# GetOverMassif/QSP-SLAM

Measured on AMD Instinct MI355X. Metric: joint-opt iters/sec (BA+SDF), higher is better.
Workload: dtype f32 as 2 x fp16 per operand (hi + 2^-11 lo'), 3 fp16 products per multiply-add, f32 accumulate (decoder); f64 (bundle adjustment)

## Files before the change

qsp_slam_amd/csrc/sdf_mlp.hpp:

```cpp
#pragma once
#include <hip/hip_runtime.h>
#include <stdint.h>

namespace qsp {

typedef float f32x16 __attribute__((ext_vector_type(16)));

#ifndef QSP_EXP_VARIANT
#define QSP_EXP_VARIANT 0
#endif
#if (QSP_EXP_VARIANT & 16)
__device__ unsigned long long qsp_dbg_ts[96];
__device__ unsigned long long qsp_dbg_rt[96];
__device__ int qsp_dbg_n;
#define QSP_TS()                                                                        \
    if (blockIdx.x == 0 && blockIdx.y == 0 && threadIdx.x == 0 && ts_n < 96) {          \
        qsp_dbg_rt[ts_n] = __builtin_amdgcn_s_memrealtime();                            \
        qsp_dbg_ts[ts_n++] = __builtin_readcyclecounter();                              \
        qsp_dbg_n = ts_n;                                                               \
    }
#define QSP_TSK(i)                                                                      \
    if (blockIdx.x == 0 && threadIdx.x == 0 && tsk_first) {                             \
        qsp_dbg_rt[80 + (i)] = __builtin_amdgcn_s_memrealtime();                        \
        qsp_dbg_ts[80 + (i)] = __builtin_readcyclecounter();                            \
    }
#else
#define QSP_TS()
#define QSP_TSK(i)
#endif

constexpr int TILE_P = 64;
constexpr int HID = 512;
constexpr int CODE_LEN = 64;
constexpr int NIN = CODE_LEN + 3;
constexpr int SKIP_COL = HID - NIN;
constexpr int K4 = SKIP_COL + 3;
constexpr int KG4 = K4 / 8;
constexpr int K0_PAD = 96;
constexpr int LDA = HID + 4;
constexpr int LDST = 68;
constexpr int STASH_SHIFT = 1;
static_assert((SKIP_COL - STASH_SHIFT) % 4 == 0 && STASH_SHIFT + NIN <= LDST, "stash row: aligned quads of units 444.., 67 inputs");
constexpr int LDJ = 96;
constexpr int NJ = 72;
constexpr int MLP_THREADS = 512;
constexpr int HT_TILES = 6;

struct MlpParams {
    const float4* wf[8];
    const float4* wb[8];
    const float* bias[8];
    const float* w8;
    float b8;
    const float* w0c;
    const float* w4c;
    const float4* w0x;
    const float4* wf3[8];
    const float4* wb3[8];
    const float4* wfh[8];
    const float4* wbh[8];
    const float4* wbh4s;
    int* range_flag;
    int use_tanh;
    int narrow;
    uint8_t skip[8];
    uint8_t ks_in[8];
    uint8_t ks_out[8];
    uint8_t ncb_in[8];
    uint8_t ncb_out[8];
};

__device__ __forceinline__ float mlp_output(float t, int use_tanh, float& dy) {
    float y = tanhf(t);
    dy = 1.f - y * y;
    if (use_tanh) {
        const float y2 = tanhf(y);
        dy = (1.f - y2 * y2) * dy;
        y = y2;
    }
    return y;
}

struct __attribute__((aligned(16))) MlpSmem {
    float act[TILE_P * LDA];
    float stash[TILE_P * LDST];
    float xin[TILE_P * 4];
    float code[CODE_LEN];
    float c0[HID];
    float c4[HID];
    float y[TILE_P];
    float red[8 * TILE_P];
    float rscale[TILE_P];
    float rres[TILE_P];
    float w8[HID];
    float dy[TILE_P];
};

template <bool AG>
__device__ __forceinline__ f32x16 mfma32t(float a, float b, f32x16 c) {
    if (AG) {
        asm("v_mfma_f32_32x32x2_f32 %0, %1, %2, %0" : "+a"(c) : "v"(a), "v"(b));
        return c;
    }
    return __builtin_amdgcn_mfma_f32_32x32x2f32(a, b, c, 0, 0, 0);
}
template <bool AG>
__device__ __forceinline__ void mfma_acc_settle(f32x16& c0, f32x16& c1, f32x16& c2, f32x16& c3) {
    if (AG) asm volatile("s_nop 15\n\ts_nop 7" : "+a"(c0), "+a"(c1), "+a"(c2), "+a"(c3));
}
template <bool AG>
__device__ __forceinline__ void mfma_acc_settle(f32x16& c0) {
    if (AG) asm volatile("s_nop 15\n\ts_nop 7" : "+a"(c0));
}

__device__ __forceinline__ int acc_row(int i, int lane) { return (i & 3) + 8 * (i >> 2) + 4 * (lane >> 5); }

typedef float f32x4 __attribute__((ext_vector_type(4)));
typedef const __attribute__((address_space(1))) f32x4* gptr4;

__device__ __forceinline__ f32x4 lds4(const float* p) { return *reinterpret_cast<const f32x4*>(p); }

#define QSP_MFMA_STEP_2x2(a0, a1, b0, b1)                   \
    acc[0][0] = mfma32t<AG>(b0.x, a0.x, acc[0][0]);         \
    acc[0][1] = mfma32t<AG>(b1.x, a0.x, acc[0][1]);              \
    acc[1][0] = mfma32t<AG>(b0.x, a1.x, acc[1][0]);              \
    acc[1][1] = mfma32t<AG>(b1.x, a1.x, acc[1][1]);              \
    acc[0][0] = mfma32t<AG>(b0.y, a0.y, acc[0][0]);              \
    acc[0][1] = mfma32t<AG>(b1.y, a0.y, acc[0][1]);              \
    acc[1][0] = mfma32t<AG>(b0.y, a1.y, acc[1][0]);              \
    acc[1][1] = mfma32t<AG>(b1.y, a1.y, acc[1][1]);              \
    acc[0][0] = mfma32t<AG>(b0.z, a0.z, acc[0][0]);              \
    acc[0][1] = mfma32t<AG>(b1.z, a0.z, acc[0][1]);              \
    acc[1][0] = mfma32t<AG>(b0.z, a1.z, acc[1][0]);              \
    acc[1][1] = mfma32t<AG>(b1.z, a1.z, acc[1][1]);              \
    acc[0][0] = mfma32t<AG>(b0.w, a0.w, acc[0][0]);              \
    acc[0][1] = mfma32t<AG>(b1.w, a0.w, acc[0][1]);              \
    acc[1][0] = mfma32t<AG>(b0.w, a1.w, acc[1][0]);              \
    acc[1][1] = mfma32t<AG>(b1.w, a1.w, acc[1][1]);

template <int PF>
struct WRing {
    f32x4 q0[PF], q1[PF];
};

template <int PF>
__device__ __forceinline__ void ring_prime(WRing<PF>& R, const float4* __restrict__ w0_, const float4* __restrict__ w1_, int lane) {
    gptr4 w0 = (gptr4)w0_;
    gptr4 w1 = (gptr4)w1_;
#pragma unroll
    for (int d = 0; d < PF; ++d) {
        R.q0[d] = w0[d * 64 + lane];
        R.q1[d] = w1[d * 64 + lane];
    }
}

struct BiasQuads {
    f32x4 v[2][4];
};

template <int KG, int PF, bool BIAS, bool AG>
__device__ __forceinline__ void gemm_2x2(const float* __restrict__ act, const float4* __restrict__ w0_,
                                         const float4* __restrict__ w1_, const float4* __restrict__ n0_,
                                         const float4* __restrict__ n1_, WRing<PF>& R, f32x16 (&acc)[2][2], int lane,
                                         const float* __restrict__ bias_wave, BiasQuads& bq) {
    static_assert(KG % PF == 0 && KG >= 2 * PF, "KG must be a multiple of the prefetch depth, at least twice it");
    gptr4 w0 = (gptr4)w0_;
    gptr4 w1 = (gptr4)w1_;
    gptr4 n0 = (gptr4)n0_;
    gptr4 n1 = (gptr4)n1_;
    const float* a_row0 = act + (lane & 31) * LDA + 4 * (lane >> 5);
    const float* a_row1 = a_row0 + 32 * LDA;
    f32x4 a0 = lds4(a_row0), a1 = lds4(a_row1);
#pragma nounroll
    for (int kg = 0; kg < KG - PF; kg += PF) {
#pragma unroll
        for (int d = 0; d < PF; ++d) {
            const f32x4 b0 = R.q0[d], b1 = R.q1[d];
#if (QSP_EXP_VARIANT & 8)
            R.q0[d] = w0[((kg + d + PF) & 15) * 64 + lane];
            R.q1[d] = w1[((kg + d + PF) & 15) * 64 + lane];
#elif (QSP_EXP_VARIANT & 4)
            R.q0[d] = w0[d * 64 + lane];
            R.q1[d] = w1[d * 64 + lane];
#elif !(QSP_EXP_VARIANT & 1)
            R.q0[d] = w0[(kg + d + PF) * 64 + lane];
            R.q1[d] = w1[(kg + d + PF) * 64 + lane];
#endif
#if !(QSP_EXP_VARIANT & 2)
            const f32x4 a0n = lds4(a_row0 + 8 * (kg + d + 1));
            const f32x4 a1n = lds4(a_row1 + 8 * (kg + d + 1));
#else
            const f32x4 a0n = a1, a1n = a0;
#endif
            __builtin_amdgcn_sched_barrier(0);
            QSP_MFMA_STEP_2x2(a0, a1, b0, b1)
            __builtin_amdgcn_sched_barrier(0);
            a0 = a0n;
            a1 = a1n;
        }
    }
    if (BIAS) {
        typedef const __attribute__((address_space(1))) f32x4* gq;
        gq bp = (gq)(bias_wave + 4 * (lane >> 5));
#pragma unroll
        for (int c = 0; c < 2; ++c)
#pragma unroll
            for (int g = 0; g < 4; ++g) bq.v[c][g] = bp[(32 * c + 8 * g) / 4];
    }
#pragma unroll
    for (int d = 0; d < PF; ++d) {
        const f32x4 b0 = R.q0[d], b1 = R.q1[d];
#if !(QSP_EXP_VARIANT & 1)
        R.q0[d] = n0[d * 64 + lane];
        R.q1[d] = n1[d * 64 + lane];
// ... 1110 lines not shown
            for (int j = 0; j < 8; ++j)
                pa[j & 3] = fmaf(fmaf((float)lo[j], 0.00048828125f, (float)hi[j]), j < 4 ? w0[j] : w1[j - 4], pa[j & 3]);
        }
        const float part = (pa[0] + pa[1]) + (pa[2] + pa[3]);
        if (lane < TP) s.red[wave * TP + lane] = part;
    }
    __syncthreads();
    if (tid < TP) {
        float t = P.b8;
#pragma unroll
        for (int q = 0; q < 4; ++q) t += s.red[q * TP + tid];
        float dy_;
        s.y[tid] = mlp_output(t, P.use_tanh, dy_);
        s.dy[tid] = dy_;
    }
    __syncthreads();
    QSP_HTS()
#ifdef QSP_H2_STAMPS
    if (threadIdx.x == 0 && blockIdx.x == 0) qsp_h2_nts = hts_n;
#endif
    if constexpr (BWD) {
        const bool seed_full = NARROW && P.skip[7];
#pragma unroll
        for (int r = 0; r < NR; ++r) {
            const int p = 32 * r + (lane & 31);
            const float dy = s.dy[p];
#pragma unroll
            for (int c = 0; c < NCB; ++c)
#pragma unroll
                for (int g = 0; g < 4; ++g) {
                    const int u0 = 32 * NCB * wave + 32 * c + 8 * g + 4 * h;
                    if (seed_full) {
                        const f32x4 wv = lds4(s.w8 + u0);
                        f32x4 v;
#pragma unroll
                        for (int q = 0; q < 4; ++q) v[q] = h2_mask_sel(dy * wv[q], mk[7][r][c >> 1], (c & 1) * 16 + 4 * g + q);
                        h2_store4(img, p, u0, v, amax);
                    } else {
                        f16x4 m;
#pragma unroll
                        for (int q = 0; q < 4; ++q) m[q] = (_Float16)h2_mask_sel(1.f, mk[7][r][c >> 1], (c & 1) * 16 + 4 * g + q);
                        *reinterpret_cast<f16x4*>(img + h2_at(p, u0)) = m;
                    }
                }
        }
        if (!NARROW) ringh_prime(ring, QSP_WBH(7), CS, lane);
        __syncthreads();
#define QSP_BWDH(L, KS_, NWB)                                                                                            \
  if (!(NARROW && P.skip[L])) {         \
    const bool act_ = !NARROW || cb0 < (int)P.ncb_in[L];                                                                  \
    const int cu0_ = 32 * NCB * wave;                                                                                    \
    (void)cu0_;                                                                                                          \
    _Pragma("unroll") for (int r_ = 0; r_ < NR; ++r_) _Pragma("unroll") for (int c_ = 0; c_ < NCB; ++c_)                 \
        _Pragma("unroll") for (int i_ = 0; i_ < 16; ++i_) { acc[r_][c_][i_] = 0.f; acc2[r_][c_][i_] = 0.f; }             \
    if constexpr (NARROW)                                                                                                \
        gemm_h2<KS_, PF, NCB, NR, false, false, true, (L) == 7>(img, QSP_WBH(L), CS, QSP_WBH(L), CS, ring, acc, acc2, lane,    \
                                                                act_ ? min((int)P.ks_out[L], KS_) : 0);                  \
    else                                                                                                                 \
        gemm_h2<KS_, PF, NCB, NR, HAND, true, false, (L) == 7>(img, QSP_WBH(L), CS, NWB, CS, ring, acc, acc2, lane);       \
    QSP_PIN_ACC()                                                                                                        \
    __syncthreads();                                                                                                     \
    float dyr_[NR];                                                   \
    _Pragma("unroll") for (int r_ = 0; r_ < NR; ++r_) dyr_[r_] = (L) == 7 ? s.dy[32 * r_ + (lane & 31)] : 1.f;           \
    _Pragma("unroll") for (int c_ = 0; c_ < NCB; ++c_) _Pragma("unroll") for (int g_ = 0; g_ < 4; ++g_) {                \
        const int u0_ = 32 * NCB * wave + 32 * c_ + 8 * g_ + 4 * h;                                                      \
        _Pragma("unroll") for (int r_ = 0; r_ < NR; ++r_) {                                                              \
            const int p_ = 32 * r_ + (lane & 31);                                                                      \
            f32x4 v_, raw_;                                                                                              \
            _Pragma("unroll") for (int q_ = 0; q_ < 4; ++q_) {                                                           \
                float x_ = fmaf(acc2[r_][c_][4 * g_ + q_], 0.00048828125f, acc[r_][c_][4 * g_ + q_]);                   \
                if ((L) == 7) x_ *= dyr_[r_];                                                                            \
                raw_[q_] = x_;                                                                                           \
                const float m_ = h2_mask_sel(x_, mk[(L) - 1][r_][c_ >> 1], (c_ & 1) * 16 + 4 * g_ + q_);                       \
                v_[q_] = m_;                                                                                             \
            }                                                                                                            \
             \
             \
             \
            if (!NARROW && (L) == 4 && cu0_ + 32 * c_ + 32 > SKIP_COL) {                 \
                if (u0_ + 3 >= SKIP_COL) *reinterpret_cast<f32x4*>(s.stash + p_ * LDST + (u0_ - (SKIP_COL - STASH_SHIFT))) = raw_; \
            }                                                                                                            \
            h2_store4(img, p_, u0_, v_, amax);                                                                           \
        }                                                                                                                \
        __builtin_amdgcn_sched_barrier(0);                                                                               \
    }                                                                                                                    \
    if (!NARROW && (L) > 1) ringh_prime(ring, NWB, CS, lane);      \
    __syncthreads();                                                                                                     \
  }
        QSP_BWDH(7, KSH, QSP_WBH(6))
        QSP_BWDH(6, KSH, QSP_WBH(5))
        QSP_BWDH(5, KSH, QSP_WBH(4))
        if constexpr (NARROW) {
            f32x4 sk[NR][4];
            gemm_side_h2<PF, NR, NW, NARROW>(img, P.wbh4s, wave, lane, sk, NARROW ? (int)P.ks_out[4] : KSH);
            const int c0 = side_c0<NR, NW>(wave);
#pragma unroll
            for (int r = 0; r < NR; ++r) {
                if (r >= side_count<NR, NW>(wave)) break;
                const int p = 32 * side_row<NR, NW>(wave, r) + (lane & 31);
#pragma unroll
                for (int g = 0; g < 4; ++g) {
                    const int k0 = 32 * c0 + 8 * g + 4 * h;
#pragma unroll
                    for (int q = 0; q < 4; ++q)
                        if (k0 + q < NIN) s.stash[p * LDST + STASH_SHIFT + k0 + q] = sk[r][g][q];
                }
            }
        }
        QSP_BWDH(4, KSH, QSP_WBH(3))
        QSP_BWDH(3, KS4, QSP_WBH(2))
        QSP_BWDH(2, KSH, QSP_WBH(1))
        QSP_BWDH(1, KSH, QSP_WBH(1))
#undef QSP_BWDH
        {
            constexpr int BPT = HID / NT;
            float bnext[7 * BPT];
#pragma unroll
            for (int l = 1; l < 8; ++l)
#pragma unroll
                for (int i = 0; i < BPT; ++i) bnext[BPT * (l - 1) + i] = P.bias[l][tid + i * NT];
            __builtin_amdgcn_sched_barrier(0);
            f32x4 gl[NR][4];
            gemm_side_h2<PF, NR, NW, NARROW>(img, P.wbh[0], wave, lane, gl, NARROW ? (int)P.ks_out[0] : KSH);
            const int c0 = side_c0<NR, NW>(wave);
            __syncthreads();
#pragma unroll
            for (int r = 0; r < NR; ++r) {
                if (r >= side_count<NR, NW>(wave)) break;
                const int p = 32 * side_row<NR, NW>(wave, r) + (lane & 31);
#pragma unroll
                for (int g = 0; g < 4; ++g) {
                    const int k0 = 32 * c0 + 8 * g + 4 * h;
                    if (k0 < NIN) {
                        const float* st = s.stash + p * LDST + STASH_SHIFT + k0;
                        f32x4 v;
#pragma unroll
                        for (int q = 0; q < 4; ++q) v[q] = gl[r][g][q] + (k0 + q < NIN ? st[q] : 0.f);
                        *reinterpret_cast<f32x4*>(s.act + p * LDG + k0) = v;
                    }
                }
            }
            __syncthreads();
#pragma unroll
            for (int l = 1; l < 8; ++l)
#pragma unroll
                for (int i = 0; i < BPT; ++i) bias_sh[(l - 1) * HID + tid + i * NT] = bnext[BPT * (l - 1) + i];
        }
    }
#undef QSP_WH
#undef QSP_WBH
#undef QSP_PIN_ACC
}

constexpr int H1_ROWS = 128;
constexpr int LDH1 = HID + 8;
struct __attribute__((aligned(16))) MlpSmemH1 {
    _Float16 img[H1_ROWS * LDH1 + 64];
    float bias[7 * HID];
    float c0[HID];
    float c4[HID];
    float w8[HID];
    float xin[H1_ROWS * 4];
    float y[H1_ROWS];
    float red[4 * H1_ROWS];
};

template <int PF, int NCB>
struct WRingH1 {
    f32x4 q[PF][NCB];
};
template <int PF, int NCB>
__device__ __forceinline__ void ringh1_prime(WRingH1<PF, NCB>& R, const float4* __restrict__ w_, int cs, int lane) {
    gbytes w = (gbytes)w_;
    const uint32_t voff = 16u * lane;
#pragma unroll
    for (int d = 0; d < PF; ++d)
#pragma unroll
        for (int c = 0; c < NCB; ++c) R.q[d][c] = ldw(w + ((size_t)c * cs + (d * 2) * 64) * 16, voff);
}

template <int KS, int PF, int NCB, int NR>
__device__ __forceinline__ void gemm_h1(const _Float16* __restrict__ img, const float4* __restrict__ w_, int cs,
                                        const float4* __restrict__ nw_, int ncs, WRingH1<PF, NCB>& R, f32x16 (&acc)[NR][NCB], int lane) {
    static_assert(KS % PF == 0 && KS >= 2 * PF && PF % 2 == 0 && NR % NCB == 0, "shape");
    constexpr int RPC = NR / NCB;
    gbytes w = (gbytes)w_;
    gbytes nw = (gbytes)nw_;
    uint32_t voff = 16u * lane;
    int b_idx = (lane & 31) * LDH1 + (lane >> 5) * 8;
    asm volatile("" : "+v"(voff), "+v"(b_idx));
    __builtin_amdgcn_s_waitcnt(0x0F70);
    const _Float16* b_row = img + b_idx;
    f16x8 bh[2][NR];
#pragma unroll
    for (int r = 0; r < NR; ++r) bh[0][r] = *reinterpret_cast<const f16x8*>(b_row + r * 32 * LDH1);
#pragma nounroll
    for (int ks = 0; ks < KS; ks += PF) {
        const bool more = ks + PF < KS;
        gbytes fb = more ? w + (size_t)(ks + PF) * 2 * 64 * 16 : nw;
        const size_t fcs = (size_t)(more ? cs : ncs) * 16;
#pragma unroll
        for (int d = 0; d < PF; ++d) {
            const _Float16* nb = b_row + 16 * (ks + d + 1);
#pragma unroll
            for (int c = 0; c < NCB; ++c) {
                const f16x8 wh = as_f16x8(R.q[d][c]);
#pragma unroll
                for (int r = 0; r < NR; ++r) acc[r][c] = __builtin_amdgcn_mfma_f32_32x32x16_f16(wh, bh[d & 1][r], acc[r][c], 0, 0, 0);
                __builtin_amdgcn_sched_barrier(0);
#pragma unroll
                for (int rr = 0; rr < RPC; ++rr)
                    bh[(d & 1) ^ 1][c * RPC + rr] = *reinterpret_cast<const f16x8*>(nb + (c * RPC + rr) * 32 * LDH1);
                if (c > 0) R.q[d][c - 1] = ldw(fb + (c - 1) * fcs + (size_t)(d * 2) * 64 * 16, voff);
                __builtin_amdgcn_sched_barrier(0);
            }
            R.q[d][NCB - 1] = ldw(fb + (NCB - 1) * fcs + (size_t)(d * 2) * 64 * 16, voff);
            __builtin_amdgcn_sched_barrier(0);
        }
    }
}

__device__ __forceinline__ void h1_store4(_Float16* img, int row, int u0, f32x4 v, float& amax) {
    amax = fmaxf(fmaxf(amax, fabsf(v[0])), fmaxf(fabsf(v[1]), fmaxf(fabsf(v[2]), fabsf(v[3]))));
    asm volatile("" : "+v"(amax));
    f16x4 hi;
#pragma unroll
    for (int q = 0; q < 4; ++q) hi[q] = (_Float16)v[q];
    *reinterpret_cast<f16x4*>(img + row * LDH1 + u0) = hi;
}

template <int PF, int NW = 4>
__device__ __forceinline__ void mlp_tile_h1(MlpSmemH1& s, const MlpParams* __restrict__ Pm, float& amax) {
    constexpr int NR = 4, NCB = 16 / NW;
    int tid = threadIdx.x;
    asm volatile("" : "+v"(tid));
    const int wave = __builtin_amdgcn_readfirstlane(tid >> 6);
    const int lane = tid & 63;
    const int h = lane >> 5;
    int oz;
    asm volatile("s_mov_b32 %0, 0" : "=s"(oz));
    const MlpParams& P = Pm[oz];
    f32x16 acc[NR][NCB];
    _Float16* img = s.img;
    if (tid < H1_ROWS) {
        const f32x4 x = lds4(s.xin + 4 * tid);
        f16x8 hi, z;
#pragma unroll
        for (int j = 0; j < 8; ++j) { hi[j] = (_Float16)0.f; z[j] = (_Float16)0.f; }
#pragma unroll
        for (int j = 0; j < 3; ++j) hi[j] = (_Float16)x[j];
        amax = fmaxf(amax, fmaxf(fabsf(x[0]), fmaxf(fabsf(x[1]), fabsf(x[2]))));
        _Float16* d = img + tid * LDH1;
        *reinterpret_cast<f16x8*>(d) = hi;
        *reinterpret_cast<f16x8*>(d + 8) = z;
    }
    const int cb0 = NCB * wave;
    constexpr int KSH = HID / 16, KS4 = K4 / 16, CS = KSH * 2 * 64, CS4 = KS4 * 2 * 64;
#define QSP_WH(L, KS_) (P.wfh[L] + (size_t)(cb0 * (KS_) * 2) * 64)
    WRingH1<PF, NCB> ring;
    ringh1_prime(ring, QSP_WH(1, KSH), CS, lane);
    __syncthreads();
#define QSP_FWD1(L, BIASPTR, GEMM_STMT)                                                                                  \
    _Pragma("unroll") for (int c_ = 0; c_ < NCB; ++c_) _Pragma("unroll") for (int g_ = 0; g_ < 4; ++g_) {                \
        const f32x4 bv_ = lds4((BIASPTR) + 32 * NCB * wave + 32 * c_ + 8 * g_ + 4 * h);                                  \
        _Pragma("unroll") for (int r_ = 0; r_ < NR; ++r_) _Pragma("unroll") for (int q_ = 0; q_ < 4; ++q_)               \
            acc[r_][c_][4 * g_ + q_] = bv_[q_];                                                                        \
        __builtin_amdgcn_sched_barrier(0);                                                                               \
    }                                                                                                                    \
    GEMM_STMT;                                                                                                           \
     \
     \
    _Pragma("unroll") for (int r_ = 0; r_ < NR; ++r_) _Pragma("unroll") for (int c_ = 0; c_ < NCB; ++c_)                 \
        asm volatile("" : "+a"(acc[r_][c_]));                                                                          \
    __syncthreads();                                                                                                     \
    _Pragma("unroll") for (int c_ = 0; c_ < NCB; ++c_) _Pragma("unroll") for (int g_ = 0; g_ < 4; ++g_) {                \
        const int u0_ = 32 * NCB * wave + 32 * c_ + 8 * g_ + 4 * h;                                                      \
        _Pragma("unroll") for (int r_ = 0; r_ < NR; ++r_) {                                                              \
            f32x4 v_;                                                                                                    \
            _Pragma("unroll") for (int q_ = 0; q_ < 4; ++q_) {                                                           \
                const float x_ = acc[r_][c_][4 * g_ + q_];                                                             \
                v_[q_] = x_ > 0.f ? x_ : 0.f;                                                                            \
            }                                                                                                            \
            h1_store4(img, 32 * r_ + (lane & 31), u0_, v_, amax);                                                        \
        }                                                                                                                \
        __builtin_amdgcn_sched_barrier(0);                                                                               \
    }                                                                                                                    \
    __syncthreads();
#define QSP_GEMM1(L, KS_, NXW, NKS) gemm_h1<KS_, PF, NCB, NR>(img, QSP_WH(L, KS_), (KS_) * 2 * 64, NXW, (NKS) * 2 * 64, ring, acc, lane)
    {
        gbytes w = (gbytes)QSP_WH(0, 1);
        const uint32_t voff = 16u * lane;
        const _Float16* b_row = img + (lane & 31) * LDH1 + (lane >> 5) * 8;
        QSP_FWD1(0, s.c0, {
            f16x8 bh0[NR];
            _Pragma("unroll") for (int r = 0; r < NR; ++r) bh0[r] = *reinterpret_cast<const f16x8*>(b_row + r * 32 * LDH1);
            _Pragma("unroll") for (int c = 0; c < NCB; ++c) {
                const f16x8 wh = as_f16x8(ldw(w + (size_t)(c * 2) * 64 * 16, voff));
                _Pragma("unroll") for (int r = 0; r < NR; ++r)
                    acc[r][c] = __builtin_amdgcn_mfma_f32_32x32x16_f16(wh, bh0[r], acc[r][c], 0, 0, 0);
            }
        })
    }
    QSP_FWD1(1, s.bias + 0 * HID, QSP_GEMM1(1, KSH, QSP_WH(2, KSH), KSH))
    QSP_FWD1(2, s.bias + 1 * HID, QSP_GEMM1(2, KSH, QSP_WH(3, KSH), KSH))
    QSP_FWD1(3, s.bias + 2 * HID, QSP_GEMM1(3, KSH, QSP_WH(4, KS4), KS4))
    if (tid < H1_ROWS) {
#pragma unroll
        for (int ci = 0; ci < 3; ++ci) {
            const float x = s.xin[tid * 4 + ci];
            img[tid * LDH1 + SKIP_COL + ci] = (_Float16)x;
        }
    }
    __syncthreads();
    QSP_FWD1(4, s.c4, QSP_GEMM1(4, KS4, QSP_WH(5, KSH), KSH))
    QSP_FWD1(5, s.bias + 4 * HID, QSP_GEMM1(5, KSH, QSP_WH(6, KSH), KSH))
    QSP_FWD1(6, s.bias + 5 * HID, QSP_GEMM1(6, KSH, QSP_WH(7, KSH), KSH))
    QSP_FWD1(7, s.bias + 6 * HID, QSP_GEMM1(7, KSH, QSP_WH(1, KSH), KSH))
#undef QSP_FWD1
#undef QSP_GEMM1
#undef QSP_WH
    if (NW == 4 || wave < 4) {
        const float* w = s.w8 + 128 * wave;
#pragma unroll
        for (int rr = 0; rr < 2; ++rr) {
            const _Float16* a = img + (lane + 64 * rr) * LDH1 + 128 * wave;
            float pa[4] = {0.f, 0.f, 0.f, 0.f};
#pragma unroll
            for (int g = 0; g < 16; ++g) {
                const f16x8 hi = *reinterpret_cast<const f16x8*>(a + 8 * g);
                const f32x4 w0 = lds4(w + 8 * g), w1 = lds4(w + 8 * g + 4);
#pragma unroll
                for (int j = 0; j < 8; ++j) pa[j & 3] = fmaf((float)hi[j], j < 4 ? w0[j] : w1[j - 4], pa[j & 3]);
            }
            s.red[wave * H1_ROWS + lane + 64 * rr] = (pa[0] + pa[1]) + (pa[2] + pa[3]);
        }
    }
    __syncthreads();
    if (tid < H1_ROWS) {
        float t = P.b8;
#pragma unroll
        for (int q = 0; q < 4; ++q) t += s.red[q * H1_ROWS + tid];
        float dy_;
        s.y[tid] = mlp_output(t, P.use_tanh, dy_);
    }
    __syncthreads();
}

}
```

qsp_slam_amd/csrc/sdf_refine.hip:

```cpp
#include <hip/hip_runtime.h>
#include <math.h>
#include <stdint.h>
#include <stdio.h>
#include <stdlib.h>
#include <string.h>

#include <algorithm>
#include <limits>
#include <string>
#include <mutex>
#include <vector>

#include "../../include/qsp_hip.h"
#include "common.hpp"
#include "sdf_mlp.hpp"

#include "sdf_kernels.hpp"

#ifndef QSP_JTJ_WAVES_DEFAULT
#define QSP_JTJ_WAVES_DEFAULT 8
#endif
#ifndef QSP_SCREEN_WAVES_DEFAULT
#define QSP_SCREEN_WAVES_DEFAULT 4
#endif


using namespace qsp;

struct qsp_decoder {
    int device = 0;
    hipStream_t stream = nullptr;
    MlpParams P{};
    MlpParams* Pd = nullptr;
    std::vector<void*> allocs;
    double mac_per_point = 0;
    int code_len = CODE_LEN;
    int fwd_bf3 = 0;
    int jac_bf3 = 0;
    bool fp16_ok = true;
    int tile_p = 64;
    int* range_flag_h = nullptr;
    bool narrow_capable = false;
    float screen_margin = 0.f;
    int32_t depth_staging = 1;
    int32_t screen_audit = 100;
    int64_t screen_min_samples = -1;
    int range_fallback = 1;
    int64_t n_range_fallbacks = 0;
    int64_t n_screen_fallbacks = 0;
    std::recursive_mutex mu;
    struct qsp_refine_batch* arena = nullptr;
    int64_t n_arena_reuse = 0, n_arena_create = 0;
};

struct qsp_decoder_group {
    std::vector<qsp_decoder*> m;
    std::vector<qsp_decoder*> lock_order;
    int device = 0;
    MlpParams* Pd = nullptr;
    std::vector<MlpParams> Ph;
    struct qsp_refine_batch* arena = nullptr;
    int64_t n_arena_reuse = 0, n_arena_create = 0;
};

struct F32Override {
    qsp_decoder* d;
    int fwd, jac;
    explicit F32Override(qsp_decoder* d_) : d(d_), fwd(d_->fwd_bf3), jac(d_->jac_bf3) { d->fwd_bf3 = 0; d->jac_bf3 = 0; }
    ~F32Override() { d->fwd_bf3 = fwd; d->jac_bf3 = jac; }
};

static int embed_family(const qsp_decoder_desc* desc, const std::vector<std::vector<float>>& W,
                        std::vector<std::vector<float>>& Wc, std::vector<std::vector<float>>& Bc, std::vector<int>& src) {
    const int nl = desc->n_layers, m = nl - 1, L = desc->code_len;
    if (nl < 3 || nl > 9 || L < 1 || L > CODE_LEN)
        return qsp_fail(QSP_ERR_UNSUPPORTED, "decoder family: 2..8 hidden layers and a code of 1..64 are supported");
    int s = desc->latent_in_layer;
    const bool has_skip = s >= 0;
    if (!has_skip) {
        s = -1;
        for (int c = std::max(1, m - 4); c <= std::min(4, m - 1) && s < 0; ++c)
            if (desc->out_dim[c - 1] >= 1 && desc->out_dim[c - 1] <= SKIP_COL) s = c;
        if (s < 0)
            return qsp_fail(QSP_ERR_UNSUPPORTED, "decoder family: without a latent_in layer one of the hidden layers 1..4 must be "
                                                  "at most 445 wide (it takes the place of the layer in front of the skip)");
    }
    if (s < 1 || s > 4 || s > m - 1 || m - s > 4)
        return qsp_fail(QSP_ERR_UNSUPPORTED, "decoder family: the latent_in layer needs 1..4 hidden layers in front of it and "
                                              "at most 4 from it on");
    if (desc->in_dim[0] != L + 3 || desc->out_dim[m] != 1)
        return qsp_fail(QSP_ERR_UNSUPPORTED, "decoder family: first layer takes [code | xyz], last layer has one output");
    for (int l = 0; l < m; ++l) {
        const int lim = (l == s - 1) ? SKIP_COL : HID;
        if (desc->out_dim[l] < 1 || desc->out_dim[l] > lim)
            return qsp_fail(QSP_ERR_UNSUPPORTED, "decoder family: hidden width above 512 (445 in front of the latent_in layer)");
    }
    for (int l = 1; l <= m; ++l) {
        const int expect = desc->out_dim[l - 1] + ((l == s && has_skip) ? L + 3 : 0);
        if (desc->in_dim[l] != expect) return qsp_fail(QSP_ERR_UNSUPPORTED, "decoder family: layer input widths do not chain");
    }
    auto in_c = [](int c) { return c == 0 ? NIN : HID; };
    auto out_c = [](int c) { return c == 8 ? 1 : (c == 3 ? SKIP_COL : HID); };
    Wc.assign(9, std::vector<float>());
    Bc.assign(9, std::vector<float>());
    src.assign(9, -1);
    for (int l = 0; l < s; ++l) src[l] = l;
    for (int l = s; l < m; ++l) src[4 + (l - s)] = l;
    src[8] = m;
    for (int c = 0; c < 9; ++c) {
        const int ic = in_c(c), oc = out_c(c);
        Wc[c].assign((size_t)oc * ic, 0.f);
        Bc[c].assign((size_t)oc, 0.f);
        const int l = src[c];
        if (l < 0) {
            for (int r = 0; r < oc; ++r) Wc[c][(size_t)r * ic + r] = 1.f;
            continue;
        }
        const int in = desc->in_dim[l], out = desc->out_dim[l];
        for (int o = 0; o < out; ++o) {
            Bc[c][o] = desc->bias[l][o];
            for (int k = 0; k < in; ++k) {
                int kc = k;
                if (c == 0) kc = (k < L) ? k : CODE_LEN + (k - L);
                if (c == 4 && has_skip) {
                    const int w = desc->out_dim[l - 1];
                    kc = (k < w) ? k : (k < w + L ? SKIP_COL + (k - w) : SKIP_COL + CODE_LEN + (k - w - L));
                }
                Wc[c][(size_t)o * ic + kc] = W[l][(size_t)o * in + k];
            }
        }
    }
    return QSP_OK;
}

static void equalize_gains(std::vector<std::vector<float>>& W, std::vector<std::vector<float>>& B) {
    const int in_dim[9] = {NIN, HID, HID, HID, HID, HID, HID, HID, HID};
    const int out_dim[9] = {HID, HID, HID, SKIP_COL, HID, HID, HID, HID, 1};
    float c_prev = 1.f;
    for (int l = 0; l < 8; ++l) {
        const int in = in_dim[l], out = out_dim[l];
        const int n_hidden = (l == 0) ? 0 : (l == 4 ? SKIP_COL : in);
        std::vector<double> norms;
        for (int o = 0; o < out; ++o) {
            double ss = 0;
            for (int k = 0; k < in; ++k) {
                const double v = (double)W[l][(size_t)o * in + k] / (k < n_hidden ? (double)c_prev : 1.0);
                ss += v * v;
            }
            if (ss > 0 && std::isfinite(ss)) norms.push_back(sqrt(ss));
        }
        double m = 0;
        if (!norms.empty()) {
            std::nth_element(norms.begin(), norms.begin() + norms.size() / 2, norms.end());
            m = norms[norms.size() / 2];
        }
        float c = 1.f;
        if (m > 0 && (m < 0x1p-8 || m > 0x1p8)) c = (float)ldexp(1.0, -(int)lrint(log2(m)));
        if (c != 1.f || c_prev != 1.f) {
            for (int o = 0; o < out; ++o) {
                for (int k = 0; k < in; ++k) W[l][(size_t)o * in + k] *= (k < n_hidden) ? c / c_prev : c;
                B[l][o] *= c;
            }
        }
        c_prev = c;
    }
    if (c_prev != 1.f)
        for (int k = 0; k < HID; ++k) W[8][k] /= c_prev;
}
// ... 117 lines not shown
                            if (o < out && k < 3) v = W[0][(size_t)o * in + CODE_LEN + k];
                            if (!(fabsf(v) < 65000.f)) d->fp16_ok = false;
                            const _Float16 hi = (_Float16)v;
                            const size_t base = ((size_t)cb * 2) * 64 * 8 + (size_t)lane * 8 + j;
                            ph[base] = hi;
                            ph[base + 64 * 8] = (_Float16)((v - (float)hi) * 2048.f);
                        }
                void* phd = nullptr;
                QSP_HIP(hipMalloc(&phd, ph.size() * sizeof(_Float16) + 16384));
                d->allocs.push_back(phd);
                QSP_HIP(hipMemcpy(phd, ph.data(), ph.size() * sizeof(_Float16), hipMemcpyHostToDevice));
                d->P.wfh[0] = (const float4*)phd;
            }
        } else {
            const int KG = (l == 4) ? KG4 : HID / 8;
            std::vector<float> pf((size_t)16 * KG * 64 * 4, 0.f);
            for (int cb = 0; cb < 16; ++cb)
                for (int kg = 0; kg < KG; ++kg)
                    for (int lane = 0; lane < 64; ++lane)
                        for (int e = 0; e < 4; ++e) {
                            const int o = 32 * cb + (lane & 31);
                            int k = 8 * kg + 4 * (lane >> 5) + e;
                            if (l == 4 && k >= SKIP_COL) k += CODE_LEN;
                            float v = 0.f;
                            if (o < out && k < in) v = W[l][(size_t)o * in + k];
                            pf[(((size_t)cb * KG + kg) * 64 + lane) * 4 + e] = v;
                        }
            rc = upload(pf, (const void**)&d->P.wf[l]);
            if (!rc) {
                const int KS = KG / 2;
                std::vector<uint16_t> p3((size_t)16 * KS * 3 * 64 * 8, 0);
                for (int cb = 0; cb < 16; ++cb)
                    for (int ks = 0; ks < KS; ++ks)
                        for (int lane = 0; lane < 64; ++lane)
                            for (int j = 0; j < 8; ++j) {
                                const int o = 32 * cb + (lane & 31);
                                int k = 16 * ks + 8 * (lane >> 5) + j;
                                if (l == 4 && k >= SKIP_COL) k += CODE_LEN;
                                float v = 0.f;
                                if (o < out && k < in) v = W[l][(size_t)o * in + k];
                                uint16_t hi, mid, lo;
                                bf16_split3(v, hi, mid, lo);
                                const size_t base = (((size_t)cb * KS + ks) * 3) * 64 * 8 + (size_t)lane * 8 + j;
                                p3[base] = hi;
                                p3[base + 64 * 8] = mid;
                                p3[base + 2 * 64 * 8] = lo;
                            }
                void* p3d = nullptr;
                QSP_HIP(hipMalloc(&p3d, p3.size() * sizeof(uint16_t) + 16384));
                d->allocs.push_back(p3d);
                QSP_HIP(hipMemcpy(p3d, p3.data(), p3.size() * sizeof(uint16_t), hipMemcpyHostToDevice));
                d->P.wf3[l] = (const float4*)p3d;
            }
            if (!rc) {
                const int KS = KG / 2;
                std::vector<_Float16> ph((size_t)16 * KS * 2 * 64 * 8, (_Float16)0.f);
                for (int cb = 0; cb < 16; ++cb)
                    for (int ks = 0; ks < KS; ++ks)
                        for (int lane = 0; lane < 64; ++lane)
                            for (int j = 0; j < 8; ++j) {
                                const int o = 32 * cb + (lane & 31);
                                int k = 16 * ks + 8 * (lane >> 5) + j;
                                if (l == 4 && k >= SKIP_COL) k += CODE_LEN;
                                float v = 0.f;
                                if (o < out && k < in) v = W[l][(size_t)o * in + k];
                                if (!(fabsf(v) < 65000.f)) d->fp16_ok = false;
                                const _Float16 hi = (_Float16)v;
                                const _Float16 lo = (_Float16)((v - (float)hi) * 2048.f);
                                const size_t base = (((size_t)cb * KS + ks) * 2) * 64 * 8 + (size_t)lane * 8 + j;
                                ph[base] = hi;
                                ph[base + 64 * 8] = lo;
                            }
                void* phd = nullptr;
                QSP_HIP(hipMalloc(&phd, ph.size() * sizeof(_Float16) + 16384));
                d->allocs.push_back(phd);
                QSP_HIP(hipMemcpy(phd, ph.data(), ph.size() * sizeof(_Float16), hipMemcpyHostToDevice));
                d->P.wfh[l] = (const float4*)phd;
            }
            if (!rc && l == 4) {
                std::vector<float> wc((size_t)HID * CODE_LEN);
                for (int o = 0; o < HID; ++o)
                    for (int k = 0; k < CODE_LEN; ++k) wc[(size_t)k * HID + o] = W[4][(size_t)o * in + SKIP_COL + k];
                rc = upload(wc, (const void**)&d->P.w4c);
            }
        }
        if (rc) return rc;
        const int NCB = (l == 0) ? 3 : 16;
        const int OG = HID / 8;
        std::vector<float> pb((size_t)NCB * OG * 64 * 4, 0.f);
        for (int cb = 0; cb < NCB; ++cb)
            for (int og = 0; og < OG; ++og)
                for (int lane = 0; lane < 64; ++lane)
                    for (int e = 0; e < 4; ++e) {
                        const int k = 32 * cb + (lane & 31);
                        const int o = 8 * og + 4 * (lane >> 5) + e;
                        float v = 0.f;
                        if (o < out && k < in) v = W[l][(size_t)o * in + k];
                        pb[(((size_t)cb * OG + og) * 64 + lane) * 4 + e] = v;
                    }
        rc = upload(pb, (const void**)&d->P.wb[l]);
        if (rc) return rc;
        {
            const int KS = HID / 16;
            std::vector<uint16_t> p3((size_t)NCB * KS * 3 * 64 * 8, 0);
            for (int cb = 0; cb < NCB; ++cb)
                for (int ks = 0; ks < KS; ++ks)
                    for (int lane = 0; lane < 64; ++lane)
                        for (int j = 0; j < 8; ++j) {
                            const int k = 32 * cb + (lane & 31);
                            const int o = 16 * ks + 8 * (lane >> 5) + j;
                            float v = 0.f;
                            if (o < out && k < in) v = W[l][(size_t)o * in + k];
                            uint16_t hi, mid, lo;
                            bf16_split3(v, hi, mid, lo);
                            const size_t base = (((size_t)cb * KS + ks) * 3) * 64 * 8 + (size_t)lane * 8 + j;
                            p3[base] = hi;
                            p3[base + 64 * 8] = mid;
                            p3[base + 2 * 64 * 8] = lo;
                        }
            void* p3d = nullptr;
            QSP_HIP(hipMalloc(&p3d, p3.size() * sizeof(uint16_t) + 16384));
            d->allocs.push_back(p3d);
            QSP_HIP(hipMemcpy(p3d, p3.data(), p3.size() * sizeof(uint16_t), hipMemcpyHostToDevice));
            d->P.wb3[l] = (const float4*)p3d;
        }
        {
            const int KS = HID / 16;
            std::vector<_Float16> ph((size_t)NCB * KS * 2 * 64 * 8, (_Float16)0.f);
            for (int cb = 0; cb < NCB; ++cb)
                for (int ks = 0; ks < KS; ++ks)
                    for (int lane = 0; lane < 64; ++lane)
                        for (int j = 0; j < 8; ++j) {
                            const int k = 32 * cb + (lane & 31);
                            const int o = 16 * ks + 8 * (lane >> 5) + j;
                            float v = 0.f;
                            if (o < out && k < in) v = l == 7 ? (float)((double)W[8][o] * W[l][(size_t)o * in + k]) : W[l][(size_t)o * in + k];
                            if (!(fabsf(v) < 65000.f)) d->fp16_ok = false;
                            const _Float16 hi = (_Float16)v;
                            const size_t base = (((size_t)cb * KS + ks) * 2) * 64 * 8 + (size_t)lane * 8 + j;
                            ph[base] = hi;
                            ph[base + 64 * 8] = (_Float16)((v - (float)hi) * 2048.f);
                        }
            void* phd = nullptr;
            QSP_HIP(hipMalloc(&phd, ph.size() * sizeof(_Float16) + 16384));
            d->allocs.push_back(phd);
            QSP_HIP(hipMemcpy(phd, ph.data(), ph.size() * sizeof(_Float16), hipMemcpyHostToDevice));
            d->P.wbh[l] = (const float4*)phd;
        }
        std::vector<float> bias(HID, 0.f);
        for (int o = 0; o < out; ++o) bias[o] = Bias[l][o];
        rc = upload(bias, (const void**)&d->P.bias[l]);
        if (rc) return rc;
    }
    {
        const int KS = HID / 16, in4 = in_dim[4], out4 = out_dim[4];
        std::vector<_Float16> ph((size_t)3 * KS * 2 * 64 * 8, (_Float16)0.f);
        for (int cb = 0; cb < 3; ++cb)
            for (int ks = 0; ks < KS; ++ks)
                for (int lane = 0; lane < 64; ++lane)
                    for (int j = 0; j < 8; ++j) {
                        const int ci = 32 * cb + (lane & 31);
                        const int o = 16 * ks + 8 * (lane >> 5) + j;
                        float v = 0.f;
                        if (o < out4 && ci < NIN) v = W[4][(size_t)o * in4 + SKIP_COL + ci];
                        const _Float16 hi = (_Float16)v;
                        const size_t base = (((size_t)cb * KS + ks) * 2) * 64 * 8 + (size_t)lane * 8 + j;
                        ph[base] = hi;
                        ph[base + 64 * 8] = (_Float16)((v - (float)hi) * 2048.f);
                    }
        void* phd = nullptr;
        QSP_HIP(hipMalloc(&phd, ph.size() * sizeof(_Float16) + 16384));
        d->allocs.push_back(phd);
        QSP_HIP(hipMemcpy(phd, ph.data(), ph.size() * sizeof(_Float16), hipMemcpyHostToDevice));
        d->P.wbh4s = (const float4*)phd;
    }
    std::vector<float> w8(W[8].begin(), W[8].end());
    int rc = upload(w8, (const void**)&d->P.w8);
    if (rc) return rc;
    d->P.b8 = Bias[8][0];
    QSP_HIP(hipHostMalloc((void**)&d->range_flag_h, sizeof(int), hipHostMallocMapped));
    *d->range_flag_h = 0;
    QSP_HIP(hipHostGetDevicePointer((void**)&d->P.range_flag, d->range_flag_h, 0));
    void* pd = nullptr;
    QSP_HIP(hipMalloc(&pd, sizeof(MlpParams)));
    d->allocs.push_back(pd);
    QSP_HIP(hipMemcpy(pd, &d->P, sizeof(MlpParams), hipMemcpyHostToDevice));
    d->Pd = (MlpParams*)pd;
    return QSP_OK;
}

static bool range_hit(qsp_decoder* d) {
    if (d->range_flag_h && *d->range_flag_h) {
        *d->range_flag_h = 0;
        return true;
    }
    return false;
}
static int range_error() {
    return qsp_fail(QSP_ERR_UNSUPPORTED, "split fp16: an activation or gradient of this decoder left fp16's range (65504); "
                                         "use the split-bf16 or f32 precision for it, or leave QSP_DEC_OPT_RANGE_FALLBACK on");
}
static bool range_should_fall_back(qsp_decoder* d) { return d->range_fallback && (d->fwd_bf3 == 2 || d->jac_bf3 == 2); }
static int check_range(qsp_decoder* d) { return range_hit(d) ? range_error() : QSP_OK; }

static int env_waves(const char* name, int dflt) {
    const char* e = getenv(name);
    const int v = e ? atoi(e) : 0;
    return (v == 4 || v == 8) ? v : dflt;
}
static int jtj_waves() { static const int w = env_waves("QSP_JTJ_WAVES", QSP_JTJ_WAVES_DEFAULT); return w; }
static int screen_waves() { static const int w = env_waves("QSP_SCREEN_WAVES", QSP_SCREEN_WAVES_DEFAULT); return w; }
static int jtj_waves_t32() { static const int w = env_waves("QSP_JTJ_WAVES_T32", 4); return w; }

template <class... A> struct Form { void (*fn)(A...); int threads; int lds; };
template <class Smem, class... A> static Form<A...> form(void (*fn)(A...), int threads) { return {fn, threads, (int)sizeof(Smem)}; }
template <class... A, class... B> static void launch(const Form<A...>& f, int grid, hipStream_t s, const B&... args) {
    hipLaunchKernelGGL(f.fn, dim3(grid), dim3(f.threads), f.lds, s, static_cast<A>(args)...);
}

template <bool BF3> static auto fwd_kernel(bool grp) { return form<MlpSmem>(grp ? k_mlp_fwd<BF3, true> : k_mlp_fwd<BF3, false>, MLP_THREADS); }
template <int NW> static auto fwd_h1_kernel(bool grp) { return form<MlpSmemH1>(grp ? k_mlp_fwd_h1<NW, true> : k_mlp_fwd_h1<NW, false>, 64 * NW); }
template <int NR, bool NARROW, int NW> static auto fwd_h2_kernel(bool grp) {
    return form<MlpSmem>(grp ? k_mlp_fwd_h2<NR, NARROW, NW, true> : k_mlp_fwd_h2<NR, NARROW, NW, false>, 64 * NW);
}
template <bool B3> static auto jtj_kernel(bool grp) { return form<MlpSmem>(grp ? k_mlp_jtj<B3, true> : k_mlp_jtj<B3, false>, MLP_THREADS); }
template <int NR, int NW, bool NARROW> static auto jtj_h2_kernel(bool grp) {
    return form<MlpSmem>(grp ? k_mlp_jtj_h2<NR, NW, NARROW, true> : k_mlp_jtj_h2<NR, NW, NARROW, false>, 64 * NW);
}
template <bool GRAD, bool BF3> static auto decode_kernel() { return form<MlpSmem>(k_decode<GRAD, BF3>, MLP_THREADS); }
template <bool GRAD, bool NARROW> static auto decode_h2_kernel() { return form<MlpSmem>(k_decode_h2<GRAD, NARROW>, H2_THREADS); }
template <int NW> static auto decode_screen_kernel() { return form<MlpSmemH1>(k_decode_screen<NW>, 64 * NW); }
template <bool BF3> static auto grid_decode_kernel() { return form<MlpSmem>(k_grid_decode<BF3>, MLP_THREADS); }
template <bool NARROW> static auto grid_decode_h2_kernel() { return form<MlpSmem>(k_grid_decode_h2<NARROW>, H2_THREADS); }
template <bool BF3> static auto group_grid_decode_kernel() { return form<MlpSmem>(k_group_grid_decode<BF3>, MLP_THREADS); }
template <bool NARROW> static auto group_grid_decode_h2_kernel() { return form<MlpSmem>(k_group_grid_decode_h2<NARROW>, H2_THREADS); }
static auto scan_kernel() { return form<float[SCAN_RAYS * SCAN_LD]>(k_scan, SCAN_RAYS); }

static auto fwd_form(int bf3, bool grp) { return bf3 ? fwd_kernel<true>(grp) : fwd_kernel<false>(grp); }
static auto fwd_h2_form(bool narrow, bool grp) { return narrow ? fwd_h2_kernel<2, true, 8>(grp) : fwd_h2_kernel<2, false, 4>(grp); }
static auto screen_form(int waves, bool grp) { return waves == 8 ? fwd_h1_kernel<8>(grp) : fwd_h1_kernel<4>(grp); }
static auto jtj_form(int bf3, bool grp) { return bf3 ? jtj_kernel<true>(grp) : jtj_kernel<false>(grp); }
static auto jtj_h2_form(bool narrow, int tile_p, int waves, int waves_t32, bool grp) {
    if (narrow && tile_p == 32) return jtj_h2_kernel<1, 8, true>(grp);
    if (narrow) return jtj_h2_kernel<2, 8, true>(grp);
    if (tile_p == 32 && waves_t32 == 8) return jtj_h2_kernel<1, 8, false>(grp);
    if (tile_p == 32) return jtj_h2_kernel<1, 4, false>(grp);
    if (waves == 8) return jtj_h2_kernel<2, 8, false>(grp);
    return jtj_h2_kernel<2, 4, false>(grp);
}
static auto decode_form(bool grad, int bf3, bool narrow) {
    if (bf3 == 2 && narrow) return grad ? decode_h2_kernel<true, true>() : decode_h2_kernel<false, true>();
    if (bf3 == 2) return grad ? decode_h2_kernel<true, false>() : decode_h2_kernel<false, false>();
    if (bf3) return grad ? decode_kernel<true, true>() : decode_kernel<false, true>();
    return grad ? decode_kernel<true, false>() : decode_kernel<false, false>();
}
static auto grid_decode_form(int bf3, bool narrow) {
    if (bf3 == 2) return narrow ? grid_decode_h2_kernel<true>() : grid_decode_h2_kernel<false>();
    return bf3 ? grid_decode_kernel<true>() : grid_decode_kernel<false>();
}
static auto group_grid_decode_form(int bf3, bool narrow) {
    if (bf3 == 2) return narrow ? group_grid_decode_h2_kernel<true>() : group_grid_decode_h2_kernel<false>();
    return bf3 ? group_grid_decode_kernel<true>() : group_grid_decode_kernel<false>();
}
static auto decode_screen_form(int waves) { return waves == 8 ? decode_screen_kernel<8>() : decode_screen_kernel<4>(); }

static int mlp_attr_once() {
    static bool done = false;
    if (done) return QSP_OK;
    const auto raise = [](const auto& f) {
        return hipFuncSetAttribute((const void*)f.fn, hipFuncAttributeMaxDynamicSharedMemorySize, f.lds);
    };
    for (const bool grp : {false, true}) {
        for (const int bf3 : {0, 1}) {
            QSP_HIP(raise(fwd_form(bf3, grp)));
            QSP_HIP(raise(jtj_form(bf3, grp)));
        }
        for (const int waves : {4, 8}) QSP_HIP(raise(screen_form(waves, grp)));
        for (const bool narrow : {false, true}) {
            QSP_HIP(raise(fwd_h2_form(narrow, grp)));
            for (const int tile_p : {32, 64})
                for (const int waves : {4, 8})
                    for (const int waves_t32 : {4, 8}) QSP_HIP(raise(jtj_h2_form(narrow, tile_p, waves, waves_t32, grp)));
        }
    }
    QSP_HIP(raise(scan_kernel()));
    for (const bool grad : {false, true})
        for (const int bf3 : {0, 1, 2})
            for (const bool narrow : {false, true}) QSP_HIP(raise(decode_form(grad, bf3, narrow)));
    for (const int waves : {4, 8}) QSP_HIP(raise(decode_screen_form(waves)));
    for (const int bf3 : {0, 1, 2})
        for (const bool narrow : {false, true}) {
            QSP_HIP(raise(grid_decode_form(bf3, narrow)));
            QSP_HIP(raise(group_grid_decode_form(bf3, narrow)));
        }
    done = true;
    return QSP_OK;
}

extern "C" int qsp_decoder_create(const qsp_decoder_desc* desc, int device, qsp_decoder** out) {
    if (!desc || !out || !desc->in_dim || !desc->out_dim || !desc->weight || !desc->bias)
        return qsp_fail(QSP_ERR_INVALID, "qsp_decoder_create: null argument");
    int n = 0;
    if (hipGetDeviceCount(&n) != hipSuccess || n <= 0) return qsp_fail(QSP_ERR_NO_DEVICE, "no HIP device visible");
    if (device < 0 || device >= n) return qsp_fail(QSP_ERR_INVALID, "device index out of range");
    QSP_HIP(hipSetDevice(device));
    qsp_decoder* d = new qsp_decoder();
// ... 1132 lines not shown
```

Baseline: 5503.

## Switch H1 decoder GEMMs to 16x16x32 MFMAs with new weight packing

Adds a second path for the fp16 single-pass (h1) MLP tile that uses 16x16x32 f16 MFMA instructions instead of 32x32x16, and makes it the default. Weights are repacked on the host into a new per-unit-tile, 32-wide K-slab layout (wfq), and the activation B operand and weight prefetch ring are reorganised to match. The likely aim is better issue density or register and accumulator use with smaller MFMA tiles. It costs more MFMA instructions, extra packed weight memory, and different LDS access patterns for B fragments.

```diff
diff --git a/qsp_slam_amd/csrc/h1_pack.hpp b/qsp_slam_amd/csrc/h1_pack.hpp
--- /dev/null
+++ b/qsp_slam_amd/csrc/h1_pack.hpp
@@ -0,0 +1,83 @@
+#pragma once
+#include <cstddef>
+#include <cstdint>
+#include <cstring>
+
+namespace qsp {
+namespace h1pack {
+
+constexpr int UNITS = 512, UT = UNITS / 16;
+constexpr int CODE = 64, NIN_ = CODE + 3, SKIP = UNITS - NIN_, K4_ = SKIP + 3;
+
+inline int k_extent(int layer) { return layer == 0 ? 32 : (layer == 4 ? K4_ : UNITS); }
+inline int slabs(int layer) { return k_extent(layer) / 32; }
+inline size_t halfs(int layer) { return (size_t)UNITS * k_extent(layer); }
+inline size_t total_bytes() {
+    size_t b = 0;
+    for (int l = 0; l < 8; ++l) b += halfs(l) * 2;
+    return b;
+}
+inline size_t at(int ks, int ut, int s, int lane, int j) { return (((size_t)ut * ks + s) * 64 + lane) * 8 + j; }
+inline void unit_k(int ut, int s, int lane, int j, int& unit, int& k) {
+    unit = 16 * ut + (lane & 15);
+    k = 32 * s + 8 * (lane >> 4) + j;
+}
+inline int in_column(int layer, int k) {
+    if (layer == 0) return k < 3 ? CODE + k : -1;
+    if (layer == 4) return k < SKIP ? k : k + CODE;
+    return k;
+}
+
+inline uint16_t f16_bits(float x) {
+    uint32_t u;
+    std::memcpy(&u, &x, 4);
+    const uint16_t sign = (uint16_t)((u >> 16) & 0x8000u);
+    const uint32_t a = u & 0x7fffffffu;
+    if (a > 0x7f800000u) return (uint16_t)(sign | 0x7e00u);
+    if (a >= 0x47800000u) return (uint16_t)(sign | 0x7c00u);
+    if (a >= 0x38800000u) {
+        const uint32_t r = a - 0x38000000u;
+        return (uint16_t)(sign | ((r + 0x0fffu + ((r >> 13) & 1u)) >> 13));
+    }
+    if (a < 0x33000000u) return sign;
+    const int e = (int)(a >> 23);
+    const uint32_t m = (a & 0x7fffffu) | 0x800000u;
+    const int sh = 126 - e;
+    const uint32_t q = m >> sh, rem = m & ((1u << sh) - 1u), half = 1u << (sh - 1);
+    return (uint16_t)(sign | (q + ((rem > half || (rem == half && (q & 1u))) ? 1u : 0u)));
+}
+inline float f16_value(uint16_t h) {
+    const uint32_t sign = (uint32_t)(h & 0x8000u) << 16;
+    const int e = (h >> 10) & 31;
+    const uint32_t m = h & 0x3ffu;
+    uint32_t u;
+    if (e == 31) u = sign | 0x7f800000u | (m << 13);
+    else if (e) u = sign | ((uint32_t)(e + 112) << 23) | (m << 13);
+    else if (!m) u = sign;
+    else {
+        float v = (float)m * 5.9604644775390625e-8f;
+        std::memcpy(&u, &v, 4);
+        u |= sign;
+    }
+    float x;
+    std::memcpy(&x, &u, 4);
+    return x;
+}
+
+inline void pack_layer(int layer, const float* W, int in, int out, uint16_t* dst) {
+    const int ks = slabs(layer);
+    for (int ut = 0; ut < UT; ++ut)
+        for (int s = 0; s < ks; ++s)
+            for (int lane = 0; lane < 64; ++lane)
+                for (int j = 0; j < 8; ++j) {
+                    int unit, k;
+                    unit_k(ut, s, lane, j, unit, k);
+                    const int col = in_column(layer, k);
+                    float v = 0.f;
+                    if (unit < out && col >= 0 && col < in) v = W[(size_t)unit * in + col];
+                    dst[at(ks, ut, s, lane, j)] = f16_bits(v);
+                }
+}
+
+}
+}
diff --git a/qsp_slam_amd/csrc/sdf_mlp.hpp b/qsp_slam_amd/csrc/sdf_mlp.hpp
--- a/qsp_slam_amd/csrc/sdf_mlp.hpp
+++ b/qsp_slam_amd/csrc/sdf_mlp.hpp
@@ -60,6 +60,7 @@
     const float4* wfh[8];
     const float4* wbh[8];
     const float4* wbh4s;
+    const float4* wfq[8];
     int* range_flag;
     int use_tanh;
     int narrow;
@@ -1476,6 +1477,10 @@
 #undef QSP_PIN_ACC
 }
 
+#ifndef QSP_H1_SHAPE
+#define QSP_H1_SHAPE 16
+#endif
+static_assert(QSP_H1_SHAPE == 16 || QSP_H1_SHAPE == 32, "QSP_H1_SHAPE: 16 (16x16x32 MFMAs) or 32 (32x32x16)");
 constexpr int H1_ROWS = 128;
 constexpr int LDH1 = HID + 8;
 struct __attribute__((aligned(16))) MlpSmemH1 {
@@ -1493,6 +1498,7 @@
 struct WRingH1 {
     f32x4 q[PF][NCB];
 };
+#if QSP_H1_SHAPE == 32
 template <int PF, int NCB>
 __device__ __forceinline__ void ringh1_prime(WRingH1<PF, NCB>& R, const float4* __restrict__ w_, int cs, int lane) {
     gbytes w = (gbytes)w_;
@@ -1543,6 +1549,58 @@
         }
     }
 }
+#else
+template <int PF, int NU>
+__device__ __forceinline__ void ringh1_prime(WRingH1<PF, NU>& R, const float4* __restrict__ w_, int cs, int lane) {
+    gbytes w = (gbytes)w_;
+    const uint32_t voff = 16u * lane;
+#pragma unroll
+    for (int d = 0; d < PF; ++d)
+#pragma unroll
+        for (int u = 0; u < NU; ++u) R.q[d][u] = ldw(w + ((size_t)u * cs + d * 64) * 16, voff);
+}
+
+template <int KS, int PF, int NU>
+__device__ __forceinline__ void gemm_h1(const _Float16* __restrict__ img, const float4* __restrict__ w_, int cs,
+                                        const float4* __restrict__ nw_, int ncs, WRingH1<PF, NU>& R, f32x4 (&acc)[NU][8], int lane) {
+    static_assert(KS % PF == 0 && KS >= 2 * PF && PF % 2 == 0 && 8 % NU == 0, "shape");
+    constexpr int RPU = 8 / NU;
+    gbytes w = (gbytes)w_;
+    gbytes nw = (gbytes)nw_;
+    uint32_t voff = 16u * lane;
+    int b_idx = (lane & 15) * LDH1 + (lane >> 4) * 8;
+    asm volatile("" : "+v"(voff), "+v"(b_idx));
+    __builtin_amdgcn_s_waitcnt(0x0F70);
+    const _Float16* b_row = img + b_idx;
+    f16x8 bq[2][8];
+#pragma unroll
+    for (int p = 0; p < 8; ++p) bq[0][p] = *reinterpret_cast<const f16x8*>(b_row + p * 16 * LDH1);
+#pragma nounroll
+    for (int ks = 0; ks < KS; ks += PF) {
+        const bool more = ks + PF < KS;
+        gbytes fb = more ? w + (size_t)(ks + PF) * 64 * 16 : nw;
+        const size_t fcs = (size_t)(more ? cs : ncs) * 16;
+#pragma unroll
+        for (int d = 0; d < PF; ++d) {
+            const _Float16* nb = b_row + 32 * (ks + d + 1);
+#pragma unroll
+            for (int u = 0; u < NU; ++u) {
+                const f16x8 wq = as_f16x8(R.q[d][u]);
+#pragma unroll
+                for (int p = 0; p < 8; ++p) acc[u][p] = __builtin_amdgcn_mfma_f32_16x16x32_f16(wq, bq[d & 1][p], acc[u][p], 0, 0, 0);
+                __builtin_amdgcn_sched_barrier(0);
+#pragma unroll
+                for (int rr = 0; rr < RPU; ++rr)
+                    bq[(d & 1) ^ 1][u * RPU + rr] = *reinterpret_cast<const f16x8*>(nb + (u * RPU + rr) * 16 * LDH1);
+                if (u > 0) R.q[d][u - 1] = ldw(fb + (u - 1) * fcs + (size_t)d * 64 * 16, voff);
+                __builtin_amdgcn_sched_barrier(0);
+            }
+            R.q[d][NU - 1] = ldw(fb + (NU - 1) * fcs + (size_t)d * 64 * 16, voff);
+            __builtin_amdgcn_sched_barrier(0);
+        }
+    }
+}
+#endif
 
 __device__ __forceinline__ void h1_store4(_Float16* img, int row, int u0, f32x4 v, float& amax) {
     amax = fmaxf(fmaxf(amax, fabsf(v[0])), fmaxf(fabsf(v[1]), fmaxf(fabsf(v[2]), fabsf(v[3]))));
@@ -1555,16 +1613,13 @@
 
 template <int PF, int NW = 4>
 __device__ __forceinline__ void mlp_tile_h1(MlpSmemH1& s, const MlpParams* __restrict__ Pm, float& amax) {
-    constexpr int NR = 4, NCB = 16 / NW;
     int tid = threadIdx.x;
     asm volatile("" : "+v"(tid));
     const int wave = __builtin_amdgcn_readfirstlane(tid >> 6);
     const int lane = tid & 63;
-    const int h = lane >> 5;
     int oz;
     asm volatile("s_mov_b32 %0, 0" : "=s"(oz));
     const MlpParams& P = Pm[oz];
-    f32x16 acc[NR][NCB];
     _Float16* img = s.img;
     if (tid < H1_ROWS) {
         const f32x4 x = lds4(s.xin + 4 * tid);
@@ -1576,8 +1631,13 @@
         amax = fmaxf(amax, fmaxf(fabsf(x[0]), fmaxf(fabsf(x[1]), fabsf(x[2]))));
         _Float16* d = img + tid * LDH1;
         *reinterpret_cast<f16x8*>(d) = hi;
-        *reinterpret_cast<f16x8*>(d + 8) = z;
-    }
+#pragma unroll
+        for (int c = 1; c < 4; ++c) *reinterpret_cast<f16x8*>(d + 8 * c) = z;
+    }
+#if QSP_H1_SHAPE == 32
+    constexpr int NR = 4, NCB = 16 / NW;
+    const int h = lane >> 5;
+    f32x16 acc[NR][NCB];
     const int cb0 = NCB * wave;
     constexpr int KSH = HID / 16, KS4 = K4 / 16, CS = KSH * 2 * 64, CS4 = KS4 * 2 * 64;
 #define QSP_WH(L, KS_) (P.wfh[L] + (size_t)(cb0 * (KS_) * 2) * 64)
@@ -1625,6 +1685,58 @@
             }
         })
     }
+#else
+    constexpr int NU = 32 / NW;
+    const int hq = lane >> 4;
+    f32x4 acc[NU][8];
+    const int ut0 = NU * wave;
+    constexpr int KSH = HID / 32, KS4 = K4 / 32, CS = KSH * 64;
+    static_assert(K4 % 32 == 0, "layer 4's K extent in slabs of 32");
+#define QSP_WH(L, KS_) (P.wfq[L] + (size_t)(ut0 * (KS_)) * 64)
+    WRingH1<PF, NU> ring;
+    ringh1_prime(ring, QSP_WH(1, KSH), CS, lane);
+    __syncthreads();
+#define QSP_FWD1(L, BIASPTR, GEMM_STMT)                                                                                  \
+    _Pragma("unroll") for (int u_ = 0; u_ < NU; ++u_) {                                                                  \
+        const f32x4 bv_ = lds4((BIASPTR) + 16 * NU * wave + 16 * u_ + 4 * hq);                                           \
+        _Pragma("unroll") for (int p_ = 0; p_ < 8; ++p_) acc[u_][p_] = bv_;                                            \
+        __builtin_amdgcn_sched_barrier(0);                                                                               \
+    }                                                                                                                    \
+    GEMM_STMT;                                                                                                           \
+     \
+     \
+    _Pragma("unroll") for (int u_ = 0; u_ < NU; ++u_) _Pragma("unroll") for (int p_ = 0; p_ < 8; ++p_)                   \
+        asm volatile("" : "+a"(acc[u_][p_]));                                                                          \
+    __syncthreads();                                                                                                     \
+    _Pragma("unroll") for (int u_ = 0; u_ < NU; ++u_) {                                                                  \
+        const int u0_ = 16 * NU * wave + 16 * u_ + 4 * hq;                                                               \
+        _Pragma("unroll") for (int p_ = 0; p_ < 8; ++p_) {                                                               \
+            f32x4 v_;                                                                                                    \
+            _Pragma("unroll") for (int q_ = 0; q_ < 4; ++q_) {                                                           \
+                const float x_ = acc[u_][p_][q_];                                                                      \
+                v_[q_] = x_ > 0.f ? x_ : 0.f;                                                                            \
+            }                                                                                                            \
+            h1_store4(img, 16 * p_ + (lane & 15), u0_, v_, amax);                                                        \
+        }                                                                                                                \
+        __builtin_amdgcn_sched_barrier(0);                                                                               \
+    }                                                                                                                    \
+    __syncthreads();
+#define QSP_GEMM1(L, KS_, NXW, NKS) gemm_h1<KS_, PF, NU>(img, QSP_WH(L, KS_), (KS_) * 64, NXW, (NKS) * 64, ring, acc, lane)
+    {
+        gbytes w = (gbytes)QSP_WH(0, 1);
+        const uint32_t voff = 16u * lane;
+        const _Float16* b_row = img + (lane & 15) * LDH1 + hq * 8;
+        QSP_FWD1(0, s.c0, {
+            f16x8 bq0[8];
+            _Pragma("unroll") for (int p = 0; p < 8; ++p) bq0[p] = *reinterpret_cast<const f16x8*>(b_row + p * 16 * LDH1);
+            _Pragma("unroll") for (int u = 0; u < NU; ++u) {
+                const f16x8 wq = as_f16x8(ldw(w + (size_t)u * 64 * 16, voff));
+                _Pragma("unroll") for (int p = 0; p < 8; ++p)
+                    acc[u][p] = __builtin_amdgcn_mfma_f32_16x16x32_f16(wq, bq0[p], acc[u][p], 0, 0, 0);
+            }
+        })
+    }
+#endif
     QSP_FWD1(1, s.bias + 0 * HID, QSP_GEMM1(1, KSH, QSP_WH(2, KSH), KSH))
     QSP_FWD1(2, s.bias + 1 * HID, QSP_GEMM1(2, KSH, QSP_WH(3, KSH), KSH))
     QSP_FWD1(3, s.bias + 2 * HID, QSP_GEMM1(3, KSH, QSP_WH(4, KS4), KS4))
diff --git a/qsp_slam_amd/csrc/sdf_refine.hip b/qsp_slam_amd/csrc/sdf_refine.hip
--- a/qsp_slam_amd/csrc/sdf_refine.hip
+++ b/qsp_slam_amd/csrc/sdf_refine.hip
@@ -14,6 +14,7 @@
 #include "../../include/qsp_hip.h"
 #include "common.hpp"
 #include "sdf_mlp.hpp"
+#include "h1_pack.hpp"
 
 #include "sdf_kernels.hpp"
 
@@ -437,6 +438,15 @@
         rc = upload(bias, (const void**)&d->P.bias[l]);
         if (rc) return rc;
     }
+    for (int l = 0; l < 8; ++l) {
+        std::vector<uint16_t> pq(h1pack::halfs(l));
+        h1pack::pack_layer(l, W[l].data(), in_dim[l], out_dim[l], pq.data());
+        void* pqd = nullptr;
+        QSP_HIP(hipMalloc(&pqd, pq.size() * sizeof(uint16_t) + 16384));
+        d->allocs.push_back(pqd);
+        QSP_HIP(hipMemcpy(pqd, pq.data(), pq.size() * sizeof(uint16_t), hipMemcpyHostToDevice));
+        d->P.wfq[l] = (const float4*)pqd;
+    }
     {
         const int KS = HID / 16, in4 = in_dim[4], out4 = out_dim[4];
         std::vector<_Float16> ph((size_t)3 * KS * 2 * 64 * 8, (_Float16)0.f);
```

Result: no change. 5501 (median of 2 runs) (-0.0%).
